# Fraunhofer-AISEC/rabe

Measured on AMD Instinct MI355X. Metric: ABE ops/sec (AC17 CP-ABE encrypt+decrypt), higher is better.
Workload: dtype u32

## Files before the change

### rabe_amd/csrc/engine_internal.h

```cpp
#pragma once
#include <hip/hip_runtime.h>
#include <stdio.h>
#include <stdlib.h>
#include <string.h>
#include <string>
#include <vector>

#include "../../include/rabe_hip.h"
#include "bn254/io.h"
#include "bn254/table_walk.h"
#include "bn254/coop3.h"

using namespace rabe::bn254;
#ifndef RB_G1_WAVES
#define RB_G1_WAVES 4
#endif
#ifndef RB_MIN_WAVES
#define RB_MIN_WAVES 1
#endif
#ifndef RB_G2_WAVES
#define RB_G2_WAVES 2
#endif
struct rhip_ctx {
  int device = 0;
  hipStream_t own_stream = nullptr;
  hipStream_t stream = nullptr;
  std::string err;
  int n_cu = 0;
  void* scratch = nullptr;
  size_t scratch_bytes = 0;
  void* fe_ws = nullptr;
  size_t fe_ws_bytes = 0;
  enum { N_WORK = 22 };
  void* work[N_WORK] = {};
  size_t work_bytes[N_WORK] = {};
  int pairing_mode = 0;
  void* fe_started = nullptr;
  uint32_t* walk_fail = nullptr;
  uint32_t* walk_count = nullptr;
  bool fe_waiter_poll = true;
  rhip_ctx* fe_waiter = nullptr;
  bool early_release = false;
  hipStream_t fork[2] = {nullptr, nullptr};
  hipEvent_t fork_ev[3] = {nullptr, nullptr, nullptr};
  bool timing = false;
  struct Pending { std::string name; hipEvent_t e0, e1; };
  std::vector<Pending> pending;
};
void rhip_ktime_begin(rhip_ctx* ctx, const char* name);
void rhip_ktime_end(rhip_ctx* ctx);
int32_t rhip_fail(rhip_ctx* ctx, hipError_t e, const char* what);
static inline int rhip_mode(const rhip_ctx* ctx) { return ctx->pairing_mode == 99 ? 0 : ctx->pairing_mode; }
int32_t rhip_fork(rhip_ctx* ctx);
int32_t rhip_join(rhip_ctx* ctx);
struct RhipOnFork {
  rhip_ctx* c; hipStream_t main;
  RhipOnFork(rhip_ctx* ctx, int i) : c(ctx), main(ctx->stream) { c->stream = c->fork[i]; }
  ~RhipOnFork() { c->stream = main; }
};
int32_t rhip_ensure_scratch(rhip_ctx* ctx, size_t bytes);
int32_t rhip_ensure_fe_ws(rhip_ctx* ctx, size_t bytes);
int32_t rhip_ensure_work(rhip_ctx* ctx, int slot, size_t bytes, void** out);
bool rhip_use_c3(const rhip_ctx* ctx, size_t n_pairs);
#define ktime_begin rhip_ktime_begin
#define ktime_end rhip_ktime_end
#define fail rhip_fail
#define ensure_scratch rhip_ensure_scratch
#define ensure_fe_ws rhip_ensure_fe_ws
#define KLAUNCH(ctx, NAME, ...)            \
  do {                                     \
    ktime_begin(ctx, NAME);                \
    hipLaunchKernelGGL(__VA_ARGS__);       \
    ktime_end(ctx);                        \
    LAUNCH_CHECK(ctx, NAME);               \
  } while (0)

#define HIP_TRY(ctx, call)                                   \
  do {                                                       \
    hipError_t e__ = (call);                                 \
    if (e__ != hipSuccess) return fail(ctx, e__, #call);     \
  } while (0)
#define LAUNCH_CHECK(ctx, name)                              \
  do {                                                       \
    hipError_t e__ = hipGetLastError();                      \
    if (e__ != hipSuccess) return fail(ctx, e__, name);      \
  } while (0)

#define NEED(ctx) do { if (!(ctx)) return RHIP_ERR_ARG; } while (0)
static inline unsigned blocks_for(size_t n, unsigned bs) { return (unsigned)((n + bs - 1) / bs); }

struct G1M { uint32_t l[16]; };
struct G2M { uint32_t l[32]; };
struct G1JM { uint32_t l[24]; };
struct GtM { uint32_t l[96]; };

__device__ __forceinline__ Fp ld_fp_m(const uint32_t* p) {
  Fp r;
#pragma unroll
  for (int i = 0; i < 8; i++) r.v[i] = p[i];
  return r;
}
__device__ __forceinline__ void st_fp_m(uint32_t* p, const Fp& a) {
#pragma unroll
  for (int i = 0; i < 8; i++) p[i] = a.v[i];
}
__device__ __forceinline__ Fp2 ld_fp2_m(const uint32_t* p) { return Fp2{ld_fp_m(p), ld_fp_m(p + 8)}; }
__device__ __forceinline__ void st_fp2_m(uint32_t* p, const Fp2& a) { st_fp_m(p, a.c0); st_fp_m(p + 8, a.c1); }
__device__ __forceinline__ G1Aff ld_g1_m(const G1M* p) { return G1Aff{ld_fp_m(p->l), ld_fp_m(p->l + 8)}; }
__device__ __forceinline__ void st_g1_m(G1M* p, const G1Aff& a) { st_fp_m(p->l, a.x); st_fp_m(p->l + 8, a.y); }
__device__ __forceinline__ G2Aff ld_g2_m(const G2M* p) { return G2Aff{ld_fp2_m(p->l), ld_fp2_m(p->l + 16)}; }
__device__ __forceinline__ void st_g2_m(G2M* p, const G2Aff& a) { st_fp2_m(p->l, a.x); st_fp2_m(p->l + 16, a.y); }
static __device__ __noinline__ Fp12 ld_gt_m(const GtM* p) {
  Fp12 r;
  r.c0.a0 = ld_fp2_m(p->l);      r.c0.a1 = ld_fp2_m(p->l + 16); r.c0.a2 = ld_fp2_m(p->l + 32);
  r.c1.a0 = ld_fp2_m(p->l + 48); r.c1.a1 = ld_fp2_m(p->l + 64); r.c1.a2 = ld_fp2_m(p->l + 80);
  return r;
}
static __device__ __noinline__ void st_gt_m(GtM* p, const Fp12& a) {
  st_fp2_m(p->l, a.c0.a0);      st_fp2_m(p->l + 16, a.c0.a1); st_fp2_m(p->l + 32, a.c0.a2);
  st_fp2_m(p->l + 48, a.c1.a0); st_fp2_m(p->l + 64, a.c1.a1); st_fp2_m(p->l + 80, a.c1.a2);
}
__device__ __forceinline__ void ld_scalar(uint32_t k[8], const rhip_fr* p) {
#pragma unroll
  for (int i = 0; i < 8; i++) k[i] = p->l[i];
  if (k[7] >= FrParams::mod(7)) {
    for (int t = 0; t < 5; t++) {
      uint32_t d[8], borrow = 0;
#pragma unroll
      for (int i = 0; i < 8; i++) d[i] = subb32(k[i], FrParams::mod(i), borrow);
      if (borrow) break;
#pragma unroll
      for (int i = 0; i < 8; i++) k[i] = d[i];
    }
  }
}

static __shared__ uint4 rb_facc_lds[36 * 64];
static __shared__ uint4 rb_facc_lds4[4 * 36 * 64];
template <int W> __device__ __forceinline__ uint4* rb_facc_base();
template <> __device__ __forceinline__ uint4* rb_facc_base<1>() { return rb_facc_lds + threadIdx.x; }
template <> __device__ __forceinline__ uint4* rb_facc_base<4>() { return rb_facc_lds4 + (threadIdx.x >> 6) * (36 * 64) + (threadIdx.x & 63); }
template <int W>
struct LdsHomeT {
  __device__ __forceinline__ Fp ld_fp(int q0) const {
    const uint4* p = rb_facc_base<W>() + q0 * 64;
    const uint4 a = p[0], b = p[64];
    Fp r;
    r.v[0] = a.x; r.v[1] = a.y; r.v[2] = a.z; r.v[3] = a.w;
    r.v[4] = b.x; r.v[5] = b.y; r.v[6] = b.z; r.v[7] = b.w;
    return r;
  }
  __device__ __forceinline__ void st_fp(int q0, const Fp& a) const {
    uint4* p = rb_facc_base<W>() + q0 * 64;
    p[0] = make_uint4(a.v[0], a.v[1], a.v[2], a.v[3]);
    p[64] = make_uint4(a.v[4], a.v[5], a.v[6], a.v[7]);
  }
  __device__ __forceinline__ Fp2 ld_q4(int q0) const { return Fp2{ld_fp(q0), ld_fp(q0 + 2)}; }
  __device__ __forceinline__ void st_q4(int q0, const Fp2& a) const { st_fp(q0, a.c0); st_fp(q0 + 2, a.c1); }
  __device__ __forceinline__ Fp6 ld_q12(int q0) const { return Fp6{ld_q4(q0), ld_q4(q0 + 4), ld_q4(q0 + 8)}; }
  __device__ __forceinline__ void st_q12(int q0, const Fp6& a) const { st_q4(q0, a.a0); st_q4(q0 + 4, a.a1); st_q4(q0 + 8, a.a2); }
  __device__ __forceinline__ Fp2 ld_f2(int i) const { return ld_q4(4 * i); }
  __device__ __forceinline__ void st_f2(int i, const Fp2& v) const { st_q4(4 * i, v); }
  __device__ __forceinline__ Fp6 ld_f6(int h) const { return ld_q12(12 * h); }
  __device__ __forceinline__ void st_f6(int h, const Fp6& v) const { st_q12(12 * h, v); }
  __device__ __forceinline__ Fp6 ld_x() const { return ld_q12(24); }
  __device__ __forceinline__ void st_x(const Fp6& v) const { st_q12(24, v); }
  __device__ __forceinline__ void fence() const { asm volatile("" ::: "memory"); }
};
typedef LdsHomeT<1> LdsHome;
template <class HOME>
struct DevWsT {
  uint4* base;
  size_t stride;
  __device__ __forceinline__ Fp2 ld2(const uint4* p) const {
    const uint4 q0 = p[0], q1 = p[stride], q2 = p[2 * stride], q3 = p[3 * stride];
    Fp2 c;
    c.c0.v[0] = q0.x; c.c0.v[1] = q0.y; c.c0.v[2] = q0.z; c.c0.v[3] = q0.w;
    c.c0.v[4] = q1.x; c.c0.v[5] = q1.y; c.c0.v[6] = q1.z; c.c0.v[7] = q1.w;
    c.c1.v[0] = q2.x; c.c1.v[1] = q2.y; c.c1.v[2] = q2.z; c.c1.v[3] = q2.w;
    c.c1.v[4] = q3.x; c.c1.v[5] = q3.y; c.c1.v[6] = q3.z; c.c1.v[7] = q3.w;
    return c;
  }
  __device__ __forceinline__ void st2(uint4* p, const Fp2& c) const {
    p[0] = make_uint4(c.c0.v[0], c.c0.v[1], c.c0.v[2], c.c0.v[3]);
    p[stride] = make_uint4(c.c0.v[4], c.c0.v[5], c.c0.v[6], c.c0.v[7]);
    p[2 * stride] = make_uint4(c.c1.v[0], c.c1.v[1], c.c1.v[2], c.c1.v[3]);
// ... 343 lines not shown
```

### rabe_amd/csrc/engine_jobs.hip

```cpp
#include "engine_internal.h"
#include "msm_chunks.h"

__device__ __forceinline__ Fp ld_fp_q(const uint4* p) {
  const uint4 a = p[0], b = p[1];
  Fp r;
  r.v[0] = a.x; r.v[1] = a.y; r.v[2] = a.z; r.v[3] = a.w;
  r.v[4] = b.x; r.v[5] = b.y; r.v[6] = b.z; r.v[7] = b.w;
  return r;
}
__device__ __forceinline__ void st_fp_q(uint4* p, const Fp& a) {
  p[0] = make_uint4(a.v[0], a.v[1], a.v[2], a.v[3]);
  p[1] = make_uint4(a.v[4], a.v[5], a.v[6], a.v[7]);
}
__device__ __forceinline__ G1Aff ld_g1_q(const G1M* p) { const uint4* q = (const uint4*)p; return G1Aff{ld_fp_q(q), ld_fp_q(q + 2)}; }
__device__ __forceinline__ void st_g1_q(G1M* p, const G1Aff& a) { uint4* q = (uint4*)p; st_fp_q(q, a.x); st_fp_q(q + 2, a.y); }
__device__ __forceinline__ G2Aff ld_g2_q(const G2M* p) {
  const uint4* q = (const uint4*)p;
  return G2Aff{Fp2{ld_fp_q(q), ld_fp_q(q + 2)}, Fp2{ld_fp_q(q + 4), ld_fp_q(q + 6)}};
}
__device__ __forceinline__ void st_g2_q(G2M* p, const G2Aff& a) {
  uint4* q = (uint4*)p;
  st_fp_q(q, a.x.c0); st_fp_q(q + 2, a.x.c1); st_fp_q(q + 4, a.y.c0); st_fp_q(q + 6, a.y.c1);
}
__device__ __forceinline__ size_t owner_of(const uint32_t* off, size_t n, size_t t) {
  size_t lo = 0, hi = n;
  while (hi - lo > 1) {
    const size_t mid = (lo + hi) >> 1;
    if (off[mid] <= t) lo = mid; else hi = mid;
  }
  return lo;
}
__device__ __forceinline__ bool fr_above_half(const uint32_t k[8]) {
  bool gt = false, decided = false;
#pragma unroll
  for (int i = 7; i >= 0; i--) {
    const uint32_t h = (FrParams::mod(i) >> 1) | (i < 7 ? (FrParams::mod(i + 1) << 31) : 0u);
    if (!decided && k[i] != h) { gt = k[i] > h; decided = true; }
  }
  return gt;
}
__device__ __forceinline__ void fr_negate_canon(uint32_t k[8]) {
  uint32_t borrow = 0;
#pragma unroll
  for (int i = 0; i < 8; i++) k[i] = subb32(FrParams::mod(i), k[i], borrow);
}
__device__ __forceinline__ bool fr_shorten(uint32_t k[8]) {
  if (!fr_above_half(k)) return false;
  fr_negate_canon(k);
  return true;
}

struct PairLists {
  G1M* P;
  G2M* Q;
  uint32_t* qref;
};
static int32_t alloc_pair_lists(rhip_ctx* ctx, size_t total_pairs, PairLists* pl) {
  void* p = nullptr;
  int32_t rc = rhip_ensure_work(ctx, 0, total_pairs * sizeof(G1M), &p);
  if (rc) return rc;
  pl->P = (G1M*)p;
  rc = rhip_ensure_work(ctx, 1, total_pairs * sizeof(G2M), &p);
  if (rc) return rc;
  pl->Q = (G2M*)p;
  rc = rhip_ensure_work(ctx, 2, total_pairs * sizeof(uint32_t), &p);
  if (rc) return rc;
  pl->qref = (uint32_t*)p;
  return RHIP_OK;
}

#ifndef RB_PAIRS_BLOCK
#define RB_PAIRS_BLOCK 256
#endif
__device__ __forceinline__ void scale_and_store(uint32_t* lds, bool active, G1Aff base, uint32_t k[8], bool negate, G1M* out, bool* is_inf) {
  if (fr_shorten(k)) negate = !negate;
  if (negate) base.y = neg(base.y);
  const G1Jac r = jac_mul_naf(base, k);
  const bool inf = !active || jac_is_inf(r);
  const Fp zinv = block_batch_inverse_n<RB_PAIRS_BLOCK>(lds, inf ? one<FpParams>() : r.z);
  *is_inf = inf;
  if (active && !inf) st_g1_q(out, jac_to_aff_with_zinv(r, zinv));
}

__device__ __forceinline__ void pair_lane(size_t v, size_t n_items, size_t total_pairs, const uint32_t* pair_off, uint32_t ppi, const uint32_t* tile_off, size_t* t,
                                          size_t* item, bool* active) {
  if (ppi) {
    const size_t per_tile = (size_t)64 * ppi;
    const size_t tile = v / per_tile, r = v % per_tile;
    size_t it = tile * 64 + (r & 63);
    *active = it < n_items;
    if (!*active) it = n_items - 1;
    *item = it;
    *t = it * ppi + (r >> 6);
  } else if (tile_off) {
    const size_t n_tiles = (n_items + 63) / 64;
    size_t lo = 0, hi = n_tiles;
    while (hi - lo > 1) {
      const size_t mid = (lo + hi) >> 1;
      if (tile_off[mid] <= v) lo = mid; else hi = mid;
    }
    const size_t r = v - tile_off[lo];
    size_t it = lo * 64 + (r & 63);
    const uint32_t j = (uint32_t)(r >> 6);
    bool act = v < tile_off[n_tiles] && it < n_items;
    if (it >= n_items) it = n_items - 1;
    const uint32_t p_it = pair_off[it + 1] - pair_off[it];
    act = act && j < p_it;
    *active = act;
    *item = it;
    *t = act ? (size_t)pair_off[it] + j : (p_it ? (size_t)pair_off[it] : total_pairs - 1);
    if (!act && !p_it) *item = owner_of(pair_off, n_items, *t);
  } else {
    *active = v < total_pairs;
    *t = *active ? v : total_pairs - 1;
    *item = owner_of(pair_off, n_items, *t);
  }
}
__global__ void __launch_bounds__(1024) k_tile_offsets(size_t n_items, const uint32_t* pair_off, uint32_t* tile_off) {
  __shared__ uint32_t part[1024];
  const size_t n_tiles = (n_items + 63) / 64;
  const size_t per = (n_tiles + 1023) / 1024, lo = (size_t)threadIdx.x * per, hi = lo + per < n_tiles ? lo + per : n_tiles;
  auto lanes_of = [&](size_t tile) {
    uint32_t mx = 0;
    const size_t i1 = tile * 64 + 64 < n_items ? tile * 64 + 64 : n_items;
    for (size_t i = tile * 64; i < i1; i++) { const uint32_t p = pair_off[i + 1] - pair_off[i]; mx = p > mx ? p : mx; }
    return 64u * mx;
  };
  uint32_t sum = 0;
  for (size_t k = lo; k < hi; k++) sum += lanes_of(k);
  part[threadIdx.x] = sum;
  __syncthreads();
  for (int d = 1; d < 1024; d <<= 1) {
    const uint32_t v = (int)threadIdx.x >= d ? part[threadIdx.x - d] : 0;
    __syncthreads();
    part[threadIdx.x] += v;
    __syncthreads();
  }
  uint32_t at = part[threadIdx.x] - sum;
  for (size_t k = lo; k < hi; k++) { tile_off[k] = at; at += lanes_of(k); }
  if (threadIdx.x == 1023) tile_off[n_tiles] = part[1023];
}
static inline uint32_t uniform_ppi(size_t n_items, size_t max_pairs, size_t total_pairs) {
  return (max_pairs && total_pairs == n_items * max_pairs) ? (uint32_t)max_pairs : 0u;
}
static inline size_t pair_lanes(size_t n_items, size_t total_pairs, uint32_t ppi) { return ppi ? (n_items + 63) / 64 * 64 * (size_t)ppi : total_pairs; }
static int32_t gather_lanes(rhip_ctx* ctx, size_t n_items, size_t max_pairs, size_t total_pairs, const uint32_t* pair_off, uint32_t ppi, const uint32_t** tile_off,
                            size_t* lanes) {
  *tile_off = nullptr;
  *lanes = pair_lanes(n_items, total_pairs, ppi);
  static const bool off = getenv("RABE_NO_PAIR_TILES") != nullptr;
  if (ppi || off || !pair_off || !max_pairs || n_items < 64) return RHIP_OK;
  const size_t n_tiles = (n_items + 63) / 64;
  if (n_tiles * 64 * max_pairs >= ((size_t)1 << 32)) return RHIP_OK;
  void* w = nullptr;
// ... 1962 lines not shown
__global__ void __launch_bounds__(64, RB_MIN_WAVES) k_gt_is_member(size_t n, const rhip_gt* a, uint32_t* ok, int mode) {
  const size_t i = (size_t)blockIdx.x * blockDim.x + threadIdx.x;
  if (i >= n) return;
  const Fp12 f = load_gt(a[i].l);
  const Fp12 f2 = fp12_frob_fn(f, 2);
  const Fp12 f4 = fp12_frob_fn(f2, 2);
  bool good = wire_words_canonical(a[i].l, 12) && !fp12_is_zero(f) && fp12_eq(fp12_mul_fn(f4, f), f2);
  if (good) {
    if (mode == 1) {
      uint32_t k[8];
#pragma unroll
      for (int w = 0; w < 8; w++) k[w] = FrParams::mod(w);
      k[0] -= 1u;
      good = fp12_eq(fp12_mul_fn(gt_pow_window(f, k), f), fp12_one());
    } else {
      const Fp12 h = fp12_cyclotomic_exp_u(fp12_cyclotomic_exp_u(f));
      const Fp12 h2 = fp12_cyclotomic_sqr_fn(h);
      good = fp12_eq(fp12_mul_fn(h2, fp12_cyclotomic_sqr_fn(h2)), fp12_frob_fn(f, 1));
    }
  }
  ok[i] = good ? 1u : 0u;
}
extern "C" int32_t rhip_ctx_collect_walk_verdicts(rhip_ctx* ctx, uint32_t* dev_fail, uint32_t* dev_count) {
  NEED(ctx);
  if ((dev_fail == nullptr) != (dev_count == nullptr)) return RHIP_ERR_ARG;
  ctx->walk_fail = dev_fail;
  ctx->walk_count = dev_count;
  return RHIP_OK;
}
extern "C" int32_t rhip_g2_in_subgroup_at(rhip_ctx* ctx, size_t n_idx, const uint32_t* idx, const rhip_g2* p, uint32_t* ok) {
  NEED(ctx);
  if (!n_idx) return RHIP_OK;
  if (!idx) return RHIP_ERR_ARG;
  KLAUNCH(ctx, "k_g2_in_subgroup", k_g2_in_subgroup, dim3(blocks_for(n_idx, 128)), dim3(128), 0, ctx->stream, n_idx, p, ok, 0, idx);
  return RHIP_OK;
}
extern "C" int32_t rhip_g2_in_subgroup(rhip_ctx* ctx, size_t n, const rhip_g2* p, uint32_t* ok) {
  NEED(ctx);
  if (!n) return RHIP_OK;
  static const int mode = getenv("RABE_G2_CHECK_BY_ORDER") ? 1 : 0;
  KLAUNCH(ctx, "k_g2_in_subgroup", k_g2_in_subgroup, dim3(blocks_for(n, 128)), dim3(128), 0, ctx->stream, n, p, ok, mode, (const uint32_t*)nullptr);
  return RHIP_OK;
}
extern "C" int32_t rhip_g2_in_subgroup_by_order(rhip_ctx* ctx, size_t n, const rhip_g2* p, uint32_t* ok) {
  NEED(ctx);
  if (!n) return RHIP_OK;
  KLAUNCH(ctx, "k_g2_in_subgroup", k_g2_in_subgroup, dim3(blocks_for(n, 128)), dim3(128), 0, ctx->stream, n, p, ok, 1, (const uint32_t*)nullptr);
  return RHIP_OK;
}
extern "C" int32_t rhip_gt_is_member(rhip_ctx* ctx, size_t n, const rhip_gt* a, uint32_t* ok) {
  NEED(ctx);
  if (!n) return RHIP_OK;
  static const int mode = getenv("RABE_GT_CHECK_BY_ORDER") ? 1 : 0;
  if (mode == 0 && rhip_use_c6_gt_pow(ctx, n)) return rhip_launch_gt_is_member_c6(ctx, n, a, ok);
  KLAUNCH(ctx, "k_gt_is_member", k_gt_is_member, dim3(blocks_for(n, 64)), dim3(64), 0, ctx->stream, n, a, ok, mode);
  return RHIP_OK;
}
extern "C" int32_t rhip_gt_is_member_by_order(rhip_ctx* ctx, size_t n, const rhip_gt* a, uint32_t* ok) {
  NEED(ctx);
  if (!n) return RHIP_OK;
  KLAUNCH(ctx, "k_gt_is_member", k_gt_is_member, dim3(blocks_for(n, 64)), dim3(64), 0, ctx->stream, n, a, ok, 1);
  return RHIP_OK;
}
__global__ void __launch_bounds__(256) k_flags_all(size_t n_seg, const uint32_t* seg_off, uint32_t scale, const uint32_t* flags, uint32_t* out) {
  const size_t s = (size_t)blockIdx.x * blockDim.x + threadIdx.x;
  if (s >= n_seg) return;
  uint32_t ok = 1;
  const size_t hi = (size_t)scale * seg_off[s + 1];
  for (size_t i = (size_t)scale * seg_off[s]; i < hi; i++) ok &= (flags[i] != 0) ? 1u : 0u;
  out[s] = ok;
}
extern "C" int32_t rhip_flags_all(rhip_ctx* ctx, size_t n_seg, const uint32_t* seg_off, uint32_t scale, const uint32_t* flags, uint32_t* out) {
  NEED(ctx);
  if (!n_seg) return RHIP_OK;
  if (!seg_off || !flags || !out || !scale) return RHIP_ERR_ARG;
  KLAUNCH(ctx, "k_flags_all", k_flags_all, dim3(blocks_for(n_seg, 256)), dim3(256), 0, ctx->stream, n_seg, seg_off, scale, flags, out);
  return RHIP_OK;
}

__global__ void __launch_bounds__(RB_PAIRS_BLOCK, 2) k_jobs_pairs(size_t n_items, size_t total, const uint32_t* cpair_off, const uint32_t* pair_off,
                                                                 const rhip_g1* base, const rhip_fr* scal, const rhip_g2* q, const rhip_g2* s_q,
                                                                 G1M* P, G2M* Q, uint32_t* qref) {
  __shared__ uint32_t lds[2 * 8 * RB_PAIRS_BLOCK];
  size_t t = (size_t)blockIdx.x * blockDim.x + threadIdx.x;
  const bool active = t < total;
  if (!active) t = total - 1;
  const size_t item = owner_of(cpair_off, n_items, t);
  const uint32_t j = (uint32_t)(t - cpair_off[item]);
  const uint32_t np = pair_off[item + 1] - pair_off[item];
  const bool is_sum = (j >= np);
  G1Aff b = aff_inf<Fp>();
  uint32_t k[8] = {1, 0, 0, 0, 0, 0, 0, 0};
  const rhip_g2* qs = s_q + item;
  if (!is_sum) {
    const size_t src = (size_t)pair_off[item] + j;
    b = load_g1(base[src].l);
    if (scal) ld_scalar(k, scal + src);
    qs = q + src;
  }
  bool p_inf;
  scale_and_store(lds, active && !is_sum, b, k, false, P + t, &p_inf);
  if (!active) return;
  const G2Aff qq = load_g2(qs->l);
  const bool skip = (!is_sum && p_inf) || aff_is_inf(qq);
  if (!skip) st_g2_q(Q + t, qq);
  qref[t] = skip ? RHIP_Q_SKIP : RHIP_Q_WALK;
}
__global__ void __launch_bounds__(256, RB_MIN_WAVES) k_cpair_off(size_t n_items, const uint32_t* pair_off, int with_sum, uint32_t* cpair_off) {
  const size_t i = (size_t)blockIdx.x * blockDim.x + threadIdx.x;
  if (i <= n_items) cpair_off[i] = pair_off[i] + (with_sum ? (uint32_t)i : 0u);
}
__global__ void __launch_bounds__(256, RB_MIN_WAVES) k_g1_to_mont(size_t n, const rhip_g1* in, G1M* out) {
  const size_t i = (size_t)blockIdx.x * blockDim.x + threadIdx.x;
  if (i < n) st_g1_q(out + i, load_g1(in[i].l));
}
extern "C" int32_t rhip_pairing_jobs(rhip_ctx* ctx, size_t n_items, size_t max_pairs, size_t n_pairs, const uint32_t* pair_off, const rhip_g1* base,
                                     const rhip_fr* scal, const rhip_g2* q, size_t max_terms, size_t n_terms, const uint32_t* sum_off,
                                     const rhip_g1* s_base, const rhip_fr* s_scal, const rhip_g2* s_q, const rhip_gt* lead, rhip_gt* out) {
  NEED(ctx);
  if (!n_items) return RHIP_OK;
  if (!pair_off) return RHIP_ERR_ARG;
  const bool with_sum = sum_off != nullptr;
  const size_t total = n_pairs + (with_sum ? n_items : 0);
  if (!total) return RHIP_ERR_ARG;
  PairLists pl;
  int32_t rc = alloc_pair_lists(ctx, total, &pl);
  if (rc) return rc;
  void *w_terms = nullptr, *w_masks = nullptr, *w_part = nullptr, *w_off = nullptr;
  uint32_t L = 1, C = 1;
  if (with_sum) choose_msm_chunks(ctx, n_items, max_terms ? max_terms : 1, &L, &C);
  rc = rhip_ensure_work(ctx, 7, (n_items + 1) * sizeof(uint32_t), &w_off);
  if (!rc && with_sum) rc = rhip_ensure_work(ctx, 4, (n_terms ? n_terms : 1) * sizeof(G1M), &w_terms);
  if (!rc && with_sum) rc = rhip_ensure_work(ctx, 5, (n_terms ? n_terms : 1) * 16 * sizeof(uint32_t), &w_masks);
  if (!rc && with_sum) rc = rhip_ensure_work(ctx, 6, n_items * L * sizeof(G1JM), &w_part);
  if (rc) return rc;
  uint32_t* cpo = (uint32_t*)w_off;
  KLAUNCH(ctx, "k_cpair_off", k_cpair_off, dim3(blocks_for(n_items + 1, 256)), dim3(256), 0, ctx->stream, n_items, pair_off, with_sum ? 1 : 0, cpo);
  KLAUNCH(ctx, "k_jobs_pairs", k_jobs_pairs, dim3(blocks_for(total, RB_PAIRS_BLOCK)), dim3(RB_PAIRS_BLOCK), 0, ctx->stream, n_items, total,
          (const uint32_t*)cpo, pair_off, base, scal, q, s_q, pl.P, pl.Q, pl.qref);
  if (with_sum) {
    if (n_terms) {
      KLAUNCH(ctx, "k_naf_masks", k_naf_masks, dim3(blocks_for(n_terms, 256)), dim3(256), 0, ctx->stream, n_terms, s_scal, (uint32_t*)w_masks);
      KLAUNCH(ctx, "k_g1_to_mont", k_g1_to_mont, dim3(blocks_for(n_terms, 256)), dim3(256), 0, ctx->stream, n_terms, s_base, (G1M*)w_terms);
    }
    KLAUNCH(ctx, "k_msm_partial_g1", (k_msm_partial<Fp, G1M, G1JM>), dim3(blocks_for(n_items * L, 64)), dim3(64), 0, ctx->stream, n_items, L, C,
            sum_off, sum_off, (const G1M*)w_terms, (const uint32_t*)w_masks, 0, (G1JM*)w_part);
    KLAUNCH(ctx, "k_msm_finish_g1", k_msm_finish_g1, dim3(blocks_for(n_items, RB_PAIRS_BLOCK)), dim3(RB_PAIRS_BLOCK), 0, ctx->stream, n_items, L,
            (const G1JM*)w_part, (const uint32_t*)cpo, pl.P, pl.qref);
  }
  return run_pair_lists(ctx, n_items, (const uint32_t*)cpo, max_pairs + (with_sum ? 1 : 0), total, pl, (const LineM*)nullptr, (const void*)nullptr, lead, out);
}


__global__ void __launch_bounds__(RB_PAIRS_BLOCK, 2) k_ac17_dec_pairs(size_t n_items, const rhip_g2* ct_c0, const rhip_g1* ct_c, const uint32_t* ct_row_off,
                                                                     const rhip_g2* sk_k0, const uint8_t* sk_qinf, int prepared, const rhip_g1* sk_k,
                                                                     const uint32_t* sk_row_off, const rhip_g1* sk_kp, const uint32_t* sk_idx,
                                                                     const uint32_t* ct_sel, const uint32_t* ct_sel_off, const uint32_t* sk_sel,
                                                                     const uint32_t* sk_sel_off, G1M* P, G2M* Q, uint32_t* qref) {
  __shared__ uint32_t lds[2 * 8 * RB_PAIRS_BLOCK];
  static_assert(RB_PAIRS_BLOCK % 128 == 0, "a block holds whole (side 0, side 1) wave pairs");
  const size_t v = (size_t)blockIdx.x * blockDim.x + threadIdx.x;
  const size_t total = n_items * 6;
  size_t t = 2 * ((v >> 7) * 64 + (v & 63)) + ((v >> 6) & 1);
  const bool active = t < total;
  if (!active) t = total - 2 + (t & 1);
  const size_t item = t / 6;
  const int j = (int)((t % 6) >> 1), side = (int)(t & 1);
  const uint32_t sk = sk_idx[item];
  G1Jac acc = jac_inf<Fp>();
  if (side == 0) {
    const uint32_t base = ct_row_off[item];
    for (uint32_t x = ct_sel_off[item]; x < ct_sel_off[item + 1]; x++)
      acc = jac_madd_fast(acc, load_g1(ct_c[(size_t)(base + ct_sel[x]) * 3 + j].l));
  } else {
    const uint32_t base = sk_row_off[sk];
    acc = aff_to_jac(load_g1(sk_kp[(size_t)sk * 3 + j].l));
    for (uint32_t x = sk_sel_off[item]; x < sk_sel_off[item + 1]; x++)
      acc = jac_madd_fast(acc, load_g1(sk_k[(size_t)(base + sk_sel[x]) * 3 + j].l));
    acc = jac_neg(acc);
  }
  const bool p_inf = !active || jac_is_inf(acc);
  const Fp zinv = block_batch_inverse_n<RB_PAIRS_BLOCK>(lds, p_inf ? one<FpParams>() : acc.z);
  if (!active) return;
  if (!p_inf) st_g1_q(P + t, jac_to_aff_with_zinv(acc, zinv));
  if (side == 0 && prepared) {
    const uint32_t line = sk * 3 + (uint32_t)j;
    qref[t] = (p_inf || sk_qinf[line]) ? RHIP_Q_SKIP : line;
    return;
  }
  const G2Aff q = load_g2((side == 0 ? sk_k0 + (size_t)sk * 3 + j : ct_c0 + item * 3 + j)->l);
  const bool skip = p_inf || aff_is_inf(q);
  if (!skip) st_g2_q(Q + t, q);
  qref[t] = skip ? RHIP_Q_SKIP : RHIP_Q_WALK;
}
static int32_t ac17_decrypt_shared(rhip_ctx* ctx, size_t n_items, const rhip_g2* ct_c0, const rhip_g1* ct_c, const uint32_t* ct_row_off,
                                   const rhip_gt* ct_cp, const rhip_g2* sk_k0, const rhip_ac17_sk_lines* sk_lines, const rhip_g1* sk_k,
                                   const uint32_t* sk_row_off, const rhip_g1* sk_kp, const uint32_t* sk_idx, const uint32_t* ct_sel,
                                   const uint32_t* ct_sel_off, const uint32_t* sk_sel, const uint32_t* sk_sel_off, rhip_gt* out) {
  PairLists pl;
  int32_t rc = alloc_pair_lists(ctx, n_items * 6, &pl);
  if (rc) return rc;
  KLAUNCH(ctx, "k_ac17_dec_pairs", k_ac17_dec_pairs, dim3(blocks_for((n_items * 3 + 63) / 64 * 128, RB_PAIRS_BLOCK)), dim3(RB_PAIRS_BLOCK), 0, ctx->stream, n_items, ct_c0, ct_c,
          ct_row_off, sk_k0, (const uint8_t*)(sk_lines ? sk_lines->q_inf : nullptr), sk_lines ? 1 : 0, sk_k, sk_row_off, sk_kp, sk_idx, ct_sel, ct_sel_off,
          sk_sel, sk_sel_off, pl.P, pl.Q, pl.qref);
  return run_pair_lists(ctx, n_items, (const uint32_t*)nullptr, 6, 0, pl, sk_lines ? (const LineM*)sk_lines->lines : (const LineM*)nullptr, sk_lines ? sk_lines->lines29 : nullptr, ct_cp, out);
}
static int ac17_dec_path(const rhip_ctx* ctx, size_t n_items) {
  static const int forced = getenv("RABE_AC17_DEC_PATH") ? atoi(getenv("RABE_AC17_DEC_PATH")) : -1;
  if (forced >= 0) return forced;
  if (rhip_use_c6(ctx, n_items, 6)) return 0;
  return rhip_use_c3(ctx, n_items * 6) ? 1 : 0;
}
extern "C" int32_t rhip_ac17_cp_decrypt_batch(rhip_ctx* ctx, size_t n_items, const rhip_g2* ct_c0, const rhip_g1* ct_c, const uint32_t* ct_row_off,
                                              const rhip_gt* ct_cp, const rhip_g2* sk_k0, const rhip_g1* sk_k, const uint32_t* sk_row_off,
                                              const rhip_g1* sk_kp, const uint32_t* sk_idx, const uint32_t* ct_sel, const uint32_t* ct_sel_off,
                                              const uint32_t* sk_sel, const uint32_t* sk_sel_off, rhip_gt* out) {
  NEED(ctx);
  if (!n_items) return RHIP_OK;
  if (ac17_dec_path(ctx, n_items) == 1)
    return rhip_ac17_cp_decrypt_batch_lanes6(ctx, n_items, ct_c0, ct_c, ct_row_off, ct_cp, sk_k0, sk_k, sk_row_off, sk_kp, sk_idx, ct_sel, ct_sel_off, sk_sel,
                                             sk_sel_off, out);
  return ac17_decrypt_shared(ctx, n_items, ct_c0, ct_c, ct_row_off, ct_cp, sk_k0, nullptr, sk_k, sk_row_off, sk_kp, sk_idx, ct_sel, ct_sel_off, sk_sel,
                             sk_sel_off, out);
}
extern "C" int32_t rhip_ac17_cp_decrypt_batch_prepared(rhip_ctx* ctx, size_t n_items, const rhip_g2* ct_c0, const rhip_g1* ct_c,
                                                       const uint32_t* ct_row_off, const rhip_gt* ct_cp, const rhip_ac17_sk_lines* sk_lines,
                                                       const rhip_g1* sk_k, const uint32_t* sk_row_off, const rhip_g1* sk_kp, const uint32_t* sk_idx,
                                                       const uint32_t* ct_sel, const uint32_t* ct_sel_off, const uint32_t* sk_sel,
                                                       const uint32_t* sk_sel_off, rhip_gt* out) {
  NEED(ctx);
  if (!sk_lines) return RHIP_ERR_ARG;
  if (!n_items) return RHIP_OK;
  static const int forced = getenv("RABE_AC17_DEC_PATH") ? atoi(getenv("RABE_AC17_DEC_PATH")) : -1;
  if (forced == 1)
    return rhip_ac17_cp_decrypt_batch_prepared_lanes3(ctx, n_items, ct_c0, ct_c, ct_row_off, ct_cp, sk_lines, sk_k, sk_row_off, sk_kp, sk_idx, ct_sel,
                                                      ct_sel_off, sk_sel, sk_sel_off, out);
  return ac17_decrypt_shared(ctx, n_items, ct_c0, ct_c, ct_row_off, ct_cp, nullptr, sk_lines, sk_k, sk_row_off, sk_kp, sk_idx, ct_sel, ct_sel_off, sk_sel,
                             sk_sel_off, out);
}
```

Before: 1.754 million.

## Deduplicate AC17 decrypt key-side sums across items sharing key and selection

Adds a GPU hash-table pass that groups decrypt items sharing the same secret key and selected-row set. Each group's key-side G1 sum is then computed once by a cooperative 8-lane-per-unit kernel with shuffle reduction. When fewer than half the items are distinct, the pair kernel switches to one thread per side-0/side-1 couple and copies the precomputed key sum instead of recomputing it. This removes redundant G1 additions when batches reuse keys and policies. In exchange it adds a memset, two extra kernels and more workspace, which are pure overhead when items are mostly unique.

```diff
diff --git a/rabe_amd/csrc/engine_internal.h b/rabe_amd/csrc/engine_internal.h
--- a/rabe_amd/csrc/engine_internal.h
+++ b/rabe_amd/csrc/engine_internal.h
@@ -31,7 +31,7 @@
   size_t scratch_bytes = 0;
   void* fe_ws = nullptr;
   size_t fe_ws_bytes = 0;
-  enum { N_WORK = 22 };
+  enum { N_WORK = 27 };
   void* work[N_WORK] = {};
   size_t work_bytes[N_WORK] = {};
   int pairing_mode = 0;
diff --git a/rabe_amd/csrc/engine_jobs.hip b/rabe_amd/csrc/engine_jobs.hip
--- a/rabe_amd/csrc/engine_jobs.hip
+++ b/rabe_amd/csrc/engine_jobs.hip
@@ -1,5 +1,6 @@
 #include "engine_internal.h"
 #include "msm_chunks.h"
+#include "sel_classes.h"
 
 __device__ __forceinline__ Fp ld_fp_q(const uint4* p) {
   const uint4 a = p[0], b = p[1];
@@ -2268,16 +2269,81 @@
 }
 
 
+struct KeysumView {
+  const uint32_t* rep;
+  const G1M* psum;
+  const uint8_t* pinf;
+  const uint32_t* count_m1;
+};
+struct SelOpsDevice {
+  __device__ __forceinline__ uint32_t load(uint32_t* p) const { return __hip_atomic_load(p, __ATOMIC_RELAXED, __HIP_MEMORY_SCOPE_AGENT); }
+  __device__ __forceinline__ uint32_t cas(uint32_t* p, uint32_t expected, uint32_t value) const { return atomicCAS(p, expected, value); }
+};
+__global__ void __launch_bounds__(256, RB_MIN_WAVES) k_ac17_sel_classes(size_t n_items, const uint32_t* sk_idx, const uint32_t* sk_sel, const uint32_t* sk_sel_off,
+                                                                       uint32_t hash_bits, size_t mask, uint32_t* table, uint32_t* rep, uint32_t* leaders) {
+  const size_t i = (size_t)blockIdx.x * blockDim.x + threadIdx.x;
+  if (i >= n_items) return;
+  const uint32_t r = rb_sel_classify(table, mask, sk_idx, sk_sel, sk_sel_off, (uint32_t)i, hash_bits, SelOpsDevice{});
+  rep[i] = r;
+  if (r == (uint32_t)i) leaders[atomicAdd(table + mask + 1, 1u) + 1u] = (uint32_t)i;
+}
+__device__ __forceinline__ bool keysum_shared(const uint32_t* count_m1, size_t n_items) { return 2 * ((size_t)*count_m1 + 1) < n_items; }
+__device__ __forceinline__ G1Jac shfl_down_jac(const G1Jac& a, int d) { return G1Jac{shfl_down_fp(a.x, d), shfl_down_fp(a.y, d), shfl_down_fp(a.z, d)}; }
+#define RB_KEYSUM_LANES 8
+__global__ void __launch_bounds__(RB_PAIRS_BLOCK, 2) k_ac17_keysum(size_t n_items, const rhip_g1* sk_k, const uint32_t* sk_row_off, const rhip_g1* sk_kp,
+                                                                  const uint32_t* sk_idx, const uint32_t* sk_sel, const uint32_t* sk_sel_off,
+                                                                  const uint32_t* leaders, const uint32_t* count_m1, G1M* psum, uint8_t* pinf) {
+  __shared__ uint32_t lds[2 * 8 * RB_PAIRS_BLOCK];
+  static_assert(64 % RB_KEYSUM_LANES == 0, "a unit's lanes sit in one wave");
+  const size_t lanes = ((size_t)*count_m1 + 1) * 3 * RB_KEYSUM_LANES;
+  if (!keysum_shared(count_m1, n_items) || (size_t)blockIdx.x * blockDim.x >= lanes) return;
+  const size_t v = (size_t)blockIdx.x * blockDim.x + threadIdx.x;
+  const bool active = v < lanes;
+  const uint32_t c = (uint32_t)(v % RB_KEYSUM_LANES);
+  G1Jac acc = jac_inf<Fp>();
+  size_t dst = 0;
+  if (active) {
+    const size_t unit = v / RB_KEYSUM_LANES;
+    const size_t item = leaders[unit / 3];
+    const int j = (int)(unit % 3);
+    const uint32_t sk = sk_idx[item];
+    const uint32_t base = sk_row_off[sk];
+    dst = item * 3 + j;
+    if (c == 0) acc = aff_to_jac(load_g1(sk_kp[(size_t)sk * 3 + j].l));
+    const uint32_t lo = sk_sel_off[item], len = sk_sel_off[item + 1] - lo;
+    const uint32_t x1 = lo + (uint32_t)(((uint64_t)len * (c + 1)) / RB_KEYSUM_LANES);
+    for (uint32_t x = lo + (uint32_t)(((uint64_t)len * c) / RB_KEYSUM_LANES); x < x1; x++)
+      acc = jac_madd_fast(acc, load_g1(sk_k[(size_t)(base + sk_sel[x]) * 3 + j].l));
+  }
+#pragma unroll 1
+  for (int d = RB_KEYSUM_LANES / 2; d >= 1; d >>= 1) acc = jac_add(acc, shfl_down_jac(acc, d));
+  acc = jac_neg(acc);
+  const bool writer = active && c == 0;
+  const bool p_inf = !writer || jac_is_inf(acc);
+  const Fp zinv = block_batch_inverse_n<RB_PAIRS_BLOCK>(lds, p_inf ? one<FpParams>() : acc.z);
+  if (!writer) return;
+  pinf[dst] = p_inf ? 1 : 0;
+  if (!p_inf) st_g1_q(psum + dst, jac_to_aff_with_zinv(acc, zinv));
+}
+template <bool DEDUP>
 __global__ void __launch_bounds__(RB_PAIRS_BLOCK, 2) k_ac17_dec_pairs(size_t n_items, const rhip_g2* ct_c0, const rhip_g1* ct_c, const uint32_t* ct_row_off,
                                                                      const rhip_g2* sk_k0, const uint8_t* sk_qinf, int prepared, const rhip_g1* sk_k,
                                                                      const uint32_t* sk_row_off, const rhip_g1* sk_kp, const uint32_t* sk_idx,
                                                                      const uint32_t* ct_sel, const uint32_t* ct_sel_off, const uint32_t* sk_sel,
-                                                                     const uint32_t* sk_sel_off, G1M* P, G2M* Q, uint32_t* qref) {
+                                                                     const uint32_t* sk_sel_off, G1M* P, G2M* Q, uint32_t* qref, KeysumView ks) {
   __shared__ uint32_t lds[2 * 8 * RB_PAIRS_BLOCK];
   static_assert(RB_PAIRS_BLOCK % 128 == 0, "a block holds whole (side 0, side 1) wave pairs");
   const size_t v = (size_t)blockIdx.x * blockDim.x + threadIdx.x;
   const size_t total = n_items * 6;
   size_t t = 2 * ((v >> 7) * 64 + (v & 63)) + ((v >> 6) & 1);
+  bool couples = false;
+  if constexpr (DEDUP) {
+    couples = keysum_shared(ks.count_m1, n_items);
+    if (couples) {
+      if ((size_t)blockIdx.x * blockDim.x >= n_items * 3) return;
+      t = 2 * v;
+    }
+  }
   const bool active = t < total;
   if (!active) t = total - 2 + (t & 1);
   const size_t item = t / 6;
@@ -2299,6 +2365,15 @@
   const Fp zinv = block_batch_inverse_n<RB_PAIRS_BLOCK>(lds, p_inf ? one<FpParams>() : acc.z);
   if (!active) return;
   if (!p_inf) st_g1_q(P + t, jac_to_aff_with_zinv(acc, zinv));
+  if constexpr (DEDUP) {
+    if (couples) {
+      const size_t src = (size_t)ks.rep[item] * 3 + j;
+      const G2Aff q1 = load_g2((ct_c0 + item * 3 + j)->l);
+      const bool skip1 = ks.pinf[src] != 0 || aff_is_inf(q1);
+      if (!skip1) { st_g1_q(P + t + 1, ld_g1_q(ks.psum + src)); st_g2_q(Q + t + 1, q1); }
+      qref[t + 1] = skip1 ? RHIP_Q_SKIP : RHIP_Q_WALK;
+    }
+  }
   if (side == 0 && prepared) {
     const uint32_t line = sk * 3 + (uint32_t)j;
     qref[t] = (p_inf || sk_qinf[line]) ? RHIP_Q_SKIP : line;
@@ -2316,9 +2391,32 @@
   PairLists pl;
   int32_t rc = alloc_pair_lists(ctx, n_items * 6, &pl);
   if (rc) return rc;
-  KLAUNCH(ctx, "k_ac17_dec_pairs", k_ac17_dec_pairs, dim3(blocks_for((n_items * 3 + 63) / 64 * 128, RB_PAIRS_BLOCK)), dim3(RB_PAIRS_BLOCK), 0, ctx->stream, n_items, ct_c0, ct_c,
-          ct_row_off, sk_k0, (const uint8_t*)(sk_lines ? sk_lines->q_inf : nullptr), sk_lines ? 1 : 0, sk_k, sk_row_off, sk_kp, sk_idx, ct_sel, ct_sel_off,
-          sk_sel, sk_sel_off, pl.P, pl.Q, pl.qref);
+  static const bool dedup = !(getenv("RABE_AC17_KEYSUM_DEDUP") && atoi(getenv("RABE_AC17_KEYSUM_DEDUP")) == 0);
+  static const uint32_t hash_bits = getenv("RABE_AC17_KEYSUM_HASH_BITS") ? (uint32_t)atoi(getenv("RABE_AC17_KEYSUM_HASH_BITS")) : 64u;
+  const dim3 grid(blocks_for((n_items * 3 + 63) / 64 * 128, RB_PAIRS_BLOCK));
+  const uint8_t* q_inf = (const uint8_t*)(sk_lines ? sk_lines->q_inf : nullptr);
+  if (dedup && n_items < 0x40000000u) {
+    const size_t entries = rb_sel_table_entries(n_items);
+    void *w_table = nullptr, *w_rep = nullptr, *w_lead = nullptr, *w_psum = nullptr, *w_pinf = nullptr;
+    rc = rhip_ensure_work(ctx, 22, (entries + 1) * sizeof(uint32_t), &w_table);
+    if (!rc) rc = rhip_ensure_work(ctx, 23, n_items * sizeof(uint32_t), &w_rep);
+    if (!rc) rc = rhip_ensure_work(ctx, 24, n_items * sizeof(uint32_t), &w_lead);
+    if (!rc) rc = rhip_ensure_work(ctx, 25, n_items * 3 * sizeof(G1M), &w_psum);
+    if (!rc) rc = rhip_ensure_work(ctx, 26, n_items * 3, &w_pinf);
+    if (rc) return rc;
+    uint32_t* table = (uint32_t*)w_table;
+    HIP_TRY(ctx, hipMemsetAsync(table, 0xFF, (entries + 1) * sizeof(uint32_t), ctx->stream));
+    KLAUNCH(ctx, "k_ac17_sel_classes", k_ac17_sel_classes, dim3(blocks_for(n_items, 256)), dim3(256), 0, ctx->stream, n_items, sk_idx, sk_sel, sk_sel_off, hash_bits,
+            entries - 1, table, (uint32_t*)w_rep, (uint32_t*)w_lead);
+    KLAUNCH(ctx, "k_ac17_keysum", k_ac17_keysum, dim3(blocks_for(n_items * 3 * RB_KEYSUM_LANES / 2, RB_PAIRS_BLOCK)), dim3(RB_PAIRS_BLOCK), 0, ctx->stream, n_items, sk_k, sk_row_off, sk_kp,
+            sk_idx, sk_sel, sk_sel_off, (const uint32_t*)w_lead, (const uint32_t*)(table + entries), (G1M*)w_psum, (uint8_t*)w_pinf);
+    const KeysumView ks{(const uint32_t*)w_rep, (const G1M*)w_psum, (const uint8_t*)w_pinf, (const uint32_t*)(table + entries)};
+    KLAUNCH(ctx, "k_ac17_dec_pairs", k_ac17_dec_pairs<true>, grid, dim3(RB_PAIRS_BLOCK), 0, ctx->stream, n_items, ct_c0, ct_c, ct_row_off, sk_k0, q_inf, sk_lines ? 1 : 0,
+            sk_k, sk_row_off, sk_kp, sk_idx, ct_sel, ct_sel_off, sk_sel, sk_sel_off, pl.P, pl.Q, pl.qref, ks);
+  } else {
+    KLAUNCH(ctx, "k_ac17_dec_pairs", k_ac17_dec_pairs<false>, grid, dim3(RB_PAIRS_BLOCK), 0, ctx->stream, n_items, ct_c0, ct_c, ct_row_off, sk_k0, q_inf, sk_lines ? 1 : 0,
+            sk_k, sk_row_off, sk_kp, sk_idx, ct_sel, ct_sel_off, sk_sel, sk_sel_off, pl.P, pl.Q, pl.qref, KeysumView{nullptr, nullptr, nullptr, nullptr});
+  }
   return run_pair_lists(ctx, n_items, (const uint32_t*)nullptr, 6, 0, pl, sk_lines ? (const LineM*)sk_lines->lines : (const LineM*)nullptr, sk_lines ? sk_lines->lines29 : nullptr, ct_cp, out);
 }
 static int ac17_dec_path(const rhip_ctx* ctx, size_t n_items) {
diff --git a/rabe_amd/csrc/sel_classes.h b/rabe_amd/csrc/sel_classes.h
--- /dev/null
+++ b/rabe_amd/csrc/sel_classes.h
@@ -0,0 +1,53 @@
+#pragma once
+#include <stddef.h>
+#include <stdint.h>
+
+#if defined(__HIPCC__) || defined(__CUDACC__)
+#define RB_SEL_HD __host__ __device__
+#else
+#define RB_SEL_HD
+#endif
+
+#define RB_SEL_EMPTY 0xFFFFFFFFu
+#define RB_SEL_PROBES 32
+
+static inline RB_SEL_HD size_t rb_sel_table_entries(size_t n_items) {
+  size_t e = 2;
+  while (e < 2 * n_items) e <<= 1;
+  return e;
+}
+static inline RB_SEL_HD uint64_t rb_sel_mix(uint64_t h, uint32_t w) {
+  h = (h ^ w) * 0x9E3779B97F4A7C15ull;
+  return h ^ (h >> 29);
+}
+static inline RB_SEL_HD uint64_t rb_sel_hash(const uint32_t* sk_idx, const uint32_t* sel, const uint32_t* sel_off, size_t item, uint32_t hash_bits) {
+  const uint32_t lo = sel_off[item], hi = sel_off[item + 1];
+  uint64_t h = rb_sel_mix(0x243F6A8885A308D3ull, sk_idx[item]);
+  h = rb_sel_mix(h, hi - lo);
+  for (uint32_t x = lo; x < hi; x++) h = rb_sel_mix(h, sel[x]);
+  h ^= h >> 30; h *= 0xBF58476D1CE4E5B9ull;
+  h ^= h >> 27; h *= 0x94D049BB133111EBull;
+  h ^= h >> 31;
+  return hash_bits >= 64 ? h : (h & ((1ull << hash_bits) - 1ull));
+}
+static inline RB_SEL_HD bool rb_sel_equal(const uint32_t* sk_idx, const uint32_t* sel, const uint32_t* sel_off, size_t a, size_t b) {
+  const uint32_t la = sel_off[a], lb = sel_off[b], n = sel_off[a + 1] - la;
+  if (sk_idx[a] != sk_idx[b] || n != sel_off[b + 1] - lb) return false;
+  for (uint32_t x = 0; x < n; x++)
+    if (sel[la + x] != sel[lb + x]) return false;
+  return true;
+}
+template <class Ops>
+static inline RB_SEL_HD uint32_t rb_sel_classify(uint32_t* table, size_t mask, const uint32_t* sk_idx, const uint32_t* sel, const uint32_t* sel_off,
+                                                 uint32_t item, uint32_t hash_bits, Ops ops, bool* gave_up = nullptr) {
+  size_t slot = (size_t)rb_sel_hash(sk_idx, sel, sel_off, item, hash_bits) & mask;
+  if (gave_up) *gave_up = false;
+  for (int probe = 0; probe < RB_SEL_PROBES; probe++, slot = (slot + 1) & mask) {
+    uint32_t old = ops.load(table + slot);
+    if (old == RB_SEL_EMPTY) old = ops.cas(table + slot, RB_SEL_EMPTY, item);
+    if (old == RB_SEL_EMPTY) return item;
+    if (rb_sel_equal(sk_idx, sel, sel_off, item, old)) return old;
+  }
+  if (gave_up) *gave_up = true;
+  return item;
+}
```

Result: no change. 1.768 million (median of 6 runs) (+0.9%).
